# EndlessReform/smoltts

Hardware: AMD Instinct MI355X
Metric: Mimi frames/sec (=12.5 x RTF), greedy DualAR decode + Mimi decode to PCM (higher is better)
Workload: dtype bf16 weights, fp32 activations/accumulate, fp32 KV cache (LM); fp32 (Mimi)

## Files before the change

### smoltts_amd/csrc/argmax_dev.h

```cpp
#pragma once
#include "x3.h"

namespace smoltts {

struct Top2 {
  float v1;
  int i1;
  float v2;
};
__device__ __forceinline__ Top2 top2_merge(Top2 a, Top2 b) {
  Top2 o;
  const bool a_first = (a.v1 > b.v1) || (a.v1 == b.v1 && a.i1 < b.i1);
  if (a_first) {
    o.v1 = a.v1; o.i1 = a.i1; o.v2 = fmaxf(a.v2, b.v1);
  } else {
    o.v1 = b.v1; o.i1 = b.i1; o.v2 = fmaxf(b.v2, a.v1);
  }
  return o;
}

__device__ __forceinline__ uint32_t mix32(uint32_t x) {
  x ^= x >> 16; x *= 0x7feb352dU; x ^= x >> 15; x *= 0x846ca68bU; x ^= x >> 16;
  return x;
}
__device__ __forceinline__ float uniform01(uint64_t seed, int slot, int frame, int step, int col) {
  uint32_t h = mix32((uint32_t)seed ^ 0x9E3779B9U * (uint32_t)(slot + 1));
  h = mix32(h ^ (uint32_t)(seed >> 32) ^ 0x85EBCA6BU * (uint32_t)(frame + 1));
  h = mix32(h ^ 0xC2B2AE35U * (uint32_t)(step + 1));
  h = mix32(h ^ 0x27D4EB2FU * (uint32_t)(col + 1));
  return ((float)(h >> 8) + 0.5f) * (1.0f / 16777216.0f);
}

struct ArgmaxScratch {
  Top2 sh[4];
  Top2 sh2[4];
  int id;
};

struct FilterScratch {
  double m[2][4];
  int c[2][4];
};

template <int CTRL>
__device__ __forceinline__ uint32_t dpp_u32(uint32_t x) { return (uint32_t)__builtin_amdgcn_update_dpp(0, (int)x, CTRL, 0xF, 0xF, true); }
template <bool ROWS32>
__device__ __forceinline__ uint32_t swap_u32(uint32_t x, int lane) {
  const bool upper = (lane & (ROWS32 ? 32 : 16)) != 0;
  if (ROWS32) {
    const auto r = __builtin_amdgcn_permlane32_swap(x, x, false, false);
    return upper ? r[0] : r[1];
  }
  const auto r = __builtin_amdgcn_permlane16_swap(x, x, false, false);
  return upper ? r[0] : r[1];
}
__device__ __forceinline__ int wave_sum_i32(int x, int lane) {
  x += (int)dpp_u32<0xB1>(x);
  x += (int)dpp_u32<0x4E>(x);
  x += (int)dpp_u32<0x141>(x);
  x += (int)dpp_u32<0x140>(x);
  x += (int)swap_u32<false>(x, lane);
  x += (int)swap_u32<true>(x, lane);
  return x;
}
#define ST_F64_STEP(FETCH)                                                         \
  {                                                                                \
    const uint64_t b_ = (uint64_t)__double_as_longlong(x);                         \
    const uint32_t lo_ = FETCH((uint32_t)b_), hi_ = FETCH((uint32_t)(b_ >> 32));   \
    x += __longlong_as_double((long long)(((uint64_t)hi_ << 32) | lo_));           \
  }
__device__ __forceinline__ double wave_sum_f64(double x, int lane) {
#define ST_SWAP16(V) swap_u32<false>((V), lane)
#define ST_SWAP32(V) swap_u32<true>((V), lane)
  ST_F64_STEP(dpp_u32<0xB1>)
  ST_F64_STEP(dpp_u32<0x4E>)
  ST_F64_STEP(dpp_u32<0x141>)
  ST_F64_STEP(dpp_u32<0x140>)
  ST_F64_STEP(ST_SWAP16)
  ST_F64_STEP(ST_SWAP32)
#undef ST_SWAP16
#undef ST_SWAP32
  return x;
}
// ... 247 lines not shown
        wu = 0;
        for (int bit = 30; bit >= 0; --bit) {
          const uint32_t cand = wu | (1u << bit);
          double m = 0.0;
#define ST_ABOVE(V, Q) if (nz_bits(((V) - a.v1) * inv_t) < cand) m += (double)(Q);
#define ST_ABOVE_S(V, J) if (ord_key(V) >= tk) ST_ABOVE(V, mass_q(((V) - a.v1) * inv_t))
          if (vec) {
#pragma unroll
            for (int i = 0; i < 8; ++i) {
              ST_ABOVE(v[i].x, fq[i * 4]) ST_ABOVE(v[i].y, fq[i * 4 + 1]) ST_ABOVE(v[i].z, fq[i * 4 + 2]) ST_ABOVE(v[i].w, fq[i * 4 + 3])
            }
          } else {
            ST_SCOLS(ST_ABOVE_S)
          }
#undef ST_ABOVE_S
#undef ST_ABOVE
          if (wg_sum_f64(m, *F, round++, lane, wave) < P) wu = cand;
        }
      }
    }
    Top2 k{-INFINITY, 0x7fffffff, -INFINITY};
    float kz = 0.f;
#define ST_KEY(V, J)                                                  \
  {                                                                   \
    const float z = ((V) - a.v1) * inv_t;                   \
    if (z >= cut && (!FILTERS || nz_bits(z) <= wu)) {                 \
      const float u = uniform01(seed, key_slot, frame, sa.step, (J)); \
      const float key = z - logf(-logf(u));                           \
      if (key > k.v1) {                                               \
        k.v1 = key; k.i1 = (J);                                       \
        if constexpr (SCORE) kz = (V) - a.v1;                         \
      }                                                               \
    }                                                                 \
  }
#define ST_KEY_S(V, J) if (ord_key(V) >= tk) ST_KEY(V, J)
    if (vec) {
#pragma unroll
      for (int i = 0; i < 8; ++i) {
        const int j = tid * 4 + i * 1024;
        if (j < n_cols) { ST_KEY(v[i].x, j) ST_KEY(v[i].y, j + 1) ST_KEY(v[i].z, j + 2) ST_KEY(v[i].w, j + 3) }
      }
    } else if (FILTERS && fon) {
      ST_SCOLS(ST_KEY_S)
    } else {
      for (int j = tid; j < n_cols; j += 256) ST_KEY(ST_LFIX(row[j], j), j)
    }
#undef ST_KEY_S
#undef ST_KEY
    const int ki = k.i1;
#pragma unroll
    for (int o = 32; o > 0; o >>= 1) {
      Top2 b;
      b.v1 = __shfl_xor(k.v1, o); b.i1 = __shfl_xor(k.i1, o); b.v2 = -INFINITY;
      k = top2_merge(k, b);
    }
    if (lane == 0) S.sh2[wave] = k;
    __syncthreads();
    const Top2 w = top2_merge(top2_merge(S.sh2[0], S.sh2[1]), top2_merge(S.sh2[2], S.sh2[3]));
    a.i1 = w.i1;
    if constexpr (SCORE) {
      if (ki == w.i1) C->z = kz;
      __syncthreads();
      score_z = C->z;
    }
  }
#undef ST_SCOLS
#undef ST_SGROUP
#undef ST_LFIX
  if (a.i1 < 0 || a.i1 >= n_cols) a.i1 = 0;
  if (tid == 0) {
    if (temp <= 0.f && margin && (margin_mask == nullptr || margin_mask[r])) {
      const float gap = a.v1 - a.v2;
      if (gap < margin[r]) {
        margin[r] = gap;
        if (sa.margin_at) sa.margin_at[r] = (sa.frames ? sa.frames[r] : sa.frame_base + r) * 64 + sa.step;
      }
    }
  }
  if constexpr (SCORE)
    if (tid == 0) *lp_out = (float)((double)score_z - (log(score_s) - 40.0 * 0.6931471805599453094));
  return a.i1;
}

template <int CTRL>
__device__ __forceinline__ Top2 top2_dpp(Top2 t) {
  Top2 b;
  b.v1 = __int_as_float(__builtin_amdgcn_update_dpp(0, __float_as_int(t.v1), CTRL, 0xF, 0xF, true));
  b.i1 = __builtin_amdgcn_update_dpp(0, t.i1, CTRL, 0xF, 0xF, true);
  b.v2 = __int_as_float(__builtin_amdgcn_update_dpp(0, __float_as_int(t.v2), CTRL, 0xF, 0xF, true));
  return top2_merge(t, b);
}
template <bool ROWS32>
__device__ __forceinline__ Top2 top2_swap(Top2 t, int lane) {
  const unsigned a[3] = {__float_as_uint(t.v1), (unsigned)t.i1, __float_as_uint(t.v2)};
  unsigned o[3];
  const bool upper = (lane & (ROWS32 ? 32 : 16)) != 0;
#pragma unroll
  for (int i = 0; i < 3; ++i) {
    if (ROWS32) {
      const auto r = __builtin_amdgcn_permlane32_swap(a[i], a[i], false, false);
      o[i] = upper ? r[0] : r[1];
    } else {
      const auto r = __builtin_amdgcn_permlane16_swap(a[i], a[i], false, false);
      o[i] = upper ? r[0] : r[1];
    }
  }
  return top2_merge(t, Top2{__uint_as_float(o[0]), (int)o[1], __uint_as_float(o[2])});
}
__device__ __forceinline__ Top2 cand_pick_wave(const float* cand, int tiles, int lane) {
  Top2 t{-INFINITY, 0x7fffffff, -INFINITY};
  for (int j = lane; j < tiles; j += 64) {
    const float4 c = *reinterpret_cast<const float4*>(cand + (size_t)j * 4);
    t = top2_merge(t, Top2{c.x, __float_as_int(c.y), c.z});
  }
  t = top2_dpp<0xB1>(t);
  t = top2_dpp<0x4E>(t);
  t = top2_dpp<0x141>(t);
  t = top2_dpp<0x140>(t);
  t = top2_swap<false>(t, lane);
  t = top2_swap<true>(t, lane);
  return t;
}

struct QkvGather {
  const float* table;
  const float* rope;
  float* q_out;
  float* kc;
  float* vc;
  int n_q_heads, n_kv_heads, cache_len, pos;
};

__device__ __forceinline__ float4 rope_gathered4(float4 v, float4 cs) {
#pragma clang fp contract(off)
  const float o0 = v.x * cs.x - v.y * cs.y, o1 = v.y * cs.x + v.x * cs.y;
  const float o2 = v.z * cs.z - v.w * cs.w, o3 = v.w * cs.z + v.z * cs.w;
  return make_float4(o0, o1, o2, o3);
}

constexpr int QG_MAX = 2;
struct QkvRegs { float4 v[QG_MAX], cs[QG_MAX]; };

__device__ __forceinline__ void qkv_gather_load(const QkvGather& g, long erow, int base, QkvRegs& o) {
  const int qd = g.n_q_heads * 64, kd = g.n_kv_heads * 64, nqkv = qd + 2 * kd;
  const float* trow = g.table + erow * nqkv;
#pragma unroll
  for (int i = 0; i < QG_MAX; ++i) {
    const int n0 = base + (threadIdx.x + i * 256) * 4;
    o.v[i] = n0 < nqkv ? *reinterpret_cast<const float4*>(trow + n0) : make_float4(0.f, 0.f, 0.f, 0.f);
    o.cs[i] = n0 < qd + kd ? *reinterpret_cast<const float4*>(g.rope + ((long)g.pos * 32 + ((n0 & 63) >> 1)) * 2) : make_float4(1.f, 0.f, 1.f, 0.f);
  }
}

__device__ __forceinline__ void qkv_gather_store(const QkvGather& g, int r, int base, const QkvRegs& in) {
  const int qd = g.n_q_heads * 64, kd = g.n_kv_heads * 64, nqkv = qd + 2 * kd;
#pragma unroll
  for (int i = 0; i < QG_MAX; ++i) {
    const int n0 = base + (threadIdx.x + i * 256) * 4;
    if (n0 >= nqkv) continue;
    float4 v = in.v[i];
    if (n0 < qd + kd) v = rope_gathered4(v, in.cs[i]);
    if (n0 < qd) {
      *reinterpret_cast<float4*>(g.q_out + (long)r * qd + n0) = v;
    } else {
      const int nn = n0 - qd;
      float* dst = nn < kd ? g.kc : g.vc;
      const int h = (nn < kd ? nn : nn - kd) >> 6, d = nn & 63;
      *reinterpret_cast<float4*>(dst + (((long)r * g.n_kv_heads + h) * g.cache_len + g.pos) * 64 + d) = v;
    }
  }
}

}
```

### smoltts_amd/csrc/gemm3.hip

```cpp
#include <stdlib.h>

#include "argmax_dev.h"
#ifndef SMOLTTS_DBG_PIECES
#define SMOLTTS_DBG_PIECES 3
#endif
#ifndef SMOLTTS_DBG_PIECES_RESID
#define SMOLTTS_DBG_PIECES_RESID SMOLTTS_DBG_PIECES
#endif

namespace smoltts {

struct Gemm3Dev {
  const char* w;
  const float* wscale;
  const char* x3;
  int M, N, K;
  int w_nt;
  int f8_act;
  int half_rows;
  const float* ssq_in;
  float eps;
  const float* bias;
  const float* resid;
  float* out;
// ... 480 lines not shown
  b = __builtin_amdgcn_cvt_scalef32_pk_fp8_bf16(b, __builtin_bit_cast(bf16x2_t, v.w), 1.0f, true);
  return make_uint2(__builtin_bit_cast(unsigned, a), __builtin_bit_cast(unsigned, b));
}

template <int NTW, int EPI>
__global__ __launch_bounds__(256) void gemm3_rows_f8_kernel(Gemm3Dev p) {
  __shared__ uint2 xs[4 * 64];
  const int tid = threadIdx.x, wave = tid >> 6, lane = tid & 63;
  const int r = lane & 15, q = lane >> 4;
  const int nchunks = p.K >> 5;
  const int mtile0 = blockIdx.y * 4;
  const int tile0 = (blockIdx.x * 4 + wave) * NTW;
  const char* sp = ((mtile0 + wave) * 16 < p.M) ? p.x3 + (size_t)(mtile0 + wave) * nchunks * 3072 + lane * 16 : nullptr;
  const char* wb[NTW];
  bool wv[NTW];
#pragma unroll
  for (int t = 0; t < NTW; ++t) {
    wv[t] = (tile0 + t) * 16 < p.N;
    wb[t] = p.w + (size_t)(tile0 + t) * nchunks * 512 + lane * 8;
  }
  f32x4 acc[NTW][4];
#pragma unroll
  for (int t = 0; t < NTW; ++t)
#pragma unroll
    for (int mt = 0; mt < 4; ++mt) acc[t][mt] = (f32x4){0.f, 0.f, 0.f, 0.f};
  uint4 stage;
  uint2 wnext[NTW];
  auto fetch = [&](int c) {
    stage = sp ? *reinterpret_cast<const uint4*>(sp + (size_t)c * 3072) : make_uint4(0, 0, 0, 0);
#pragma unroll
    for (int t = 0; t < NTW; ++t) wnext[t] = wv[t] ? *reinterpret_cast<const uint2*>(wb[t] + (size_t)c * 512) : make_uint2(0, 0);
  };
  fetch(0);
  for (int c = 0; c < nchunks; ++c) {
    __syncthreads();
    xs[tid] = bf16x8_to_fp8x8(stage);
    long a[NTW];
#pragma unroll
    for (int t = 0; t < NTW; ++t) a[t] = __builtin_bit_cast(long, wnext[t]);
    __syncthreads();
    if (c + 1 < nchunks) fetch(c + 1);
#pragma unroll
    for (int mt = 0; mt < 4; ++mt) {
      const long b = __builtin_bit_cast(long, xs[mt * 64 + lane]);
#pragma unroll
      for (int t = 0; t < NTW; ++t) acc[t][mt] = __builtin_amdgcn_mfma_f32_16x16x32_fp8_fp8(a[t], b, acc[t][mt], 0, 0, 0);
    }
  }
  rows_epilogue<NTW, EPI, true>(p, acc, mtile0, tile0, r, q);
}

__device__ __forceinline__ float dpp_ror8(float x) {
  return __int_as_float(__builtin_amdgcn_update_dpp(0, __float_as_int(x), 0x128, 0xF, 0xF, true));
}
__device__ __forceinline__ float row8_sum(float x) {
  x += __int_as_float(__builtin_amdgcn_update_dpp(0, __float_as_int(x), 0xB1, 0xF, 0xF, true));
  x += __int_as_float(__builtin_amdgcn_update_dpp(0, __float_as_int(x), 0x4E, 0xF, 0xF, true));
  x += __int_as_float(__builtin_amdgcn_update_dpp(0, __float_as_int(x), 0x141, 0xF, 0xF, true));
  return x;
}
__device__ __forceinline__ void swap16(float& a, float& b) {
  const auto r = __builtin_amdgcn_permlane16_swap(__float_as_uint(a), __float_as_uint(b), false, false);
  a = __uint_as_float(r[0]);
  b = __uint_as_float(r[1]);
}
__device__ __forceinline__ void dot4x2(float4 a, float4 b, float4 k0, float4 k1, float& lo, float& hi) {
  lo = a.x * k0.x; lo = fmaf(a.y, k0.y, lo); lo = fmaf(a.z, k0.z, lo); lo = fmaf(a.w, k0.w, lo);
  hi = b.x * k1.x; hi = fmaf(b.y, k1.y, hi); hi = fmaf(b.z, k1.z, hi); hi = fmaf(b.w, k1.w, hi);
}
__device__ __forceinline__ float score16(float4 a, float4 b, float4 k0, float4 k1) {
  float lo, hi;
  dot4x2(a, b, k0, k1, lo, hi);
  return row8_sum(lo) + row8_sum(hi);
}

#ifndef SMOLTTS_DBG_AWO_ORDER
#define SMOLTTS_DBG_AWO_ORDER 1
#endif
constexpr int AWO_R = 2;

template <int G, bool TWO>
struct AwoUnit {
  float4 ka0, kb0, va0, vb0, ka1, kb1, va1, vb1, qa[G], qb[G];
  int rl, kvc;
  bool hv, ok0, ok1;
};

template <int G, bool TWO, bool PICK>
__device__ __forceinline__ void awo_load(AwoUnit<G, TWO>& u, const Gemm3Dev& p, int unit, int kv_pairs, int row0, int lane, long erow = 0,
                                         bool write_kv = false) {
  const int kq = lane >> 5, jj = (lane >> 3) & 3, hb = jj & 1, m8 = lane & 7;
  const int L = p.a_pos + 1;
  u.rl = unit / kv_pairs;
  const int kvh = (unit - u.rl * kv_pairs) * 2 + kq, row = row0 + u.rl;
  u.hv = kvh < p.n_kv_heads;
  u.kvc = u.hv ? kvh : p.n_kv_heads - 1;
  const long cb = (((long)row * p.n_kv_heads + u.kvc) * p.cache_len) * 64 + 4 * m8;
  u.ok0 = jj < L;
  u.ok1 = TWO && jj + 4 < L;
  const long o0 = cb + (long)(u.ok0 ? jj : 0) * 64, o1 = cb + (long)(u.ok1 ? jj + 4 : 0) * 64;
  const float *k0p = p.kc + o0, *v0p = p.vc + o0, *k1p = p.kc + o1, *v1p = p.vc + o1;
  const int qd = p.n_q_heads * 64, kd = p.n_kv_heads * 64;
  const float* trow = PICK ? p.pk_table + erow * (qd + 2 * kd) : nullptr;
  const bool new0 = PICK && jj == p.a_pos, new1 = PICK && TWO && jj + 4 == p.a_pos;
  if (PICK) {
    const float *tk = trow + qd + u.kvc * 64 + 4 * m8, *tv = trow + qd + kd + u.kvc * 64 + 4 * m8;
    if (new0) { k0p = tk; v0p = tv; }
    if (new1) { k1p = tk; v1p = tv; }
  }
  u.ka0 = *reinterpret_cast<const float4*>(k0p); u.kb0 = *reinterpret_cast<const float4*>(k0p + 32);
  u.va0 = *reinterpret_cast<const float4*>(v0p + 32 * hb); u.vb0 = *reinterpret_cast<const float4*>(v0p + 32 * (1 - hb));
  if (TWO) {
    u.ka1 = *reinterpret_cast<const float4*>(k1p); u.kb1 = *reinterpret_cast<const float4*>(k1p + 32);
    u.va1 = *reinterpret_cast<const float4*>(v1p + 32 * hb); u.vb1 = *reinterpret_cast<const float4*>(v1p + 32 * (1 - hb));
  }
#pragma unroll
  for (int g = 0; g < G; ++g) {
    const float* qp = PICK ? trow + (u.kvc * G + g) * 64 + 4 * m8 : p.aq + (long)row * qd + (u.kvc * G + g) * 64 + 4 * m8;
    u.qa[g] = *reinterpret_cast<const float4*>(qp);
    u.qb[g] = *reinterpret_cast<const float4*>(qp + 32);
  }
  if (PICK) {
    const float4 csa = *reinterpret_cast<const float4*>(p.pk_rope + ((long)p.a_pos * 32 + 2 * m8) * 2);
    const float4 csb = *reinterpret_cast<const float4*>(p.pk_rope + ((long)p.a_pos * 32 + 16 + 2 * m8) * 2);
#pragma unroll
    for (int g = 0; g < G; ++g) { u.qa[g] = rope_gathered4(u.qa[g], csa); u.qb[g] = rope_gathered4(u.qb[g], csb); }
    const float4 ra0 = rope_gathered4(u.ka0, csa), rb0 = rope_gathered4(u.kb0, csb);
    if (new0) { u.ka0 = ra0; u.kb0 = rb0; }
    if (TWO) {
      const float4 ra1 = rope_gathered4(u.ka1, csa), rb1 = rope_gathered4(u.kb1, csb);
      if (new1) { u.ka1 = ra1; u.kb1 = rb1; }
    }
    if (write_kv && u.hv && (new0 || new1)) {
      float* kw = p.kc + cb + (long)p.a_pos * 64;
      float* vw = p.vc + cb + (long)p.a_pos * 64;
      const float4 ka = new0 ? u.ka0 : u.ka1, kb = new0 ? u.kb0 : u.kb1, va = new0 ? u.va0 : u.va1, vb = new0 ? u.vb0 : u.vb1;
      *reinterpret_cast<float4*>(kw) = ka; *reinterpret_cast<float4*>(kw + 32) = kb;
      *reinterpret_cast<float4*>(vw + 32 * hb) = va; *reinterpret_cast<float4*>(vw + 32 * (1 - hb)) = vb;
    }
  }
}

template <int G, bool TWO>
__device__ __forceinline__ void awo_compute(const AwoUnit<G, TWO>& u, char* frag, int lane) {
#pragma clang fp contract(off)
  constexpr int R = AWO_R;
  const int hb = (lane >> 3) & 1, m8 = lane & 7;
  const bool up = (lane & 16) != 0;
#pragma unroll
  for (int g = 0; g < G; ++g) {
    const float4 a = make_float4(u.qa[g].x * 0.125f, u.qa[g].y * 0.125f, u.qa[g].z * 0.125f, u.qa[g].w * 0.125f);
    const float4 b = make_float4(u.qb[g].x * 0.125f, u.qb[g].y * 0.125f, u.qb[g].z * 0.125f, u.qb[g].w * 0.125f);
    float s0 = score16(a, b, u.ka0, u.kb0), s1 = -INFINITY;
    s0 = u.ok0 ? s0 : -INFINITY;
    if (TWO) {
      s1 = score16(a, b, u.ka1, u.kb1);
      s1 = u.ok1 ? s1 : -INFINITY;
    }
    float mx = TWO ? fmaxf(s0, s1) : s0;
    mx = fmaxf(mx, dpp_ror8(mx));
    {
      float t = mx;
      swap16(mx, t);
      mx = fmaxf(mx, t);
    }
    const float e0 = __expf(s0 - mx);
    float den = e0;
    float4 oa = make_float4(e0 * u.va0.x, e0 * u.va0.y, e0 * u.va0.z, e0 * u.va0.w);
    float4 ob = make_float4(e0 * u.vb0.x, e0 * u.vb0.y, e0 * u.vb0.z, e0 * u.vb0.w);
    if (TWO) {
      const float e1 = __expf(s1 - mx);
      den += e1;
      oa.x = fmaf(e1, u.va1.x, oa.x); oa.y = fmaf(e1, u.va1.y, oa.y); oa.z = fmaf(e1, u.va1.z, oa.z); oa.w = fmaf(e1, u.va1.w, oa.w);
      ob.x = fmaf(e1, u.vb1.x, ob.x); ob.y = fmaf(e1, u.vb1.y, ob.y); ob.z = fmaf(e1, u.vb1.z, ob.z); ob.w = fmaf(e1, u.vb1.w, ob.w);
    }
    den += dpp_ror8(den);
    {
      float t = den;
      swap16(den, t);
      den += t;
    }
    oa.x += dpp_ror8(ob.x); oa.y += dpp_ror8(ob.y); oa.z += dpp_ror8(ob.z); oa.w += dpp_ror8(ob.w);
    swap16(oa.x, oa.z);
    swap16(oa.y, oa.w);
    const float inv = 1.0f / den;
    const float ox = (oa.x + oa.z) * inv, oy = (oa.y + oa.w) * inv;
    uint32_t h, mm, l;
    split3_pair(ox, oy, h, mm, l);
    const int c = 2 * (u.kvc * G + g) + hb;
    char* fp = frag + ((size_t)((c * 3) * 4 + (m8 >> 1)) * R + u.rl) * 16 + (m8 & 1) * 8 + (up ? 4 : 0);
    if (u.hv) {
      *reinterpret_cast<uint32_t*>(fp) = h;
      *reinterpret_cast<uint32_t*>(fp + 4 * R * 16) = mm;
      *reinterpret_cast<uint32_t*>(fp + 8 * R * 16) = l;
    }
  }
}

constexpr int AWO_NA = 4, AWO_NB = 8, AWO_U = 3;

template <int G, int T, bool TWO, bool W8, bool PICK, int NBF>
__global__ __launch_bounds__(768) void attn_wo_kernel(const char* w_, const float* kc_, const float* vc_, const float* q_or_cand, const float* pk_table_,
                                                      int m_tiles, int N_, int K_, int heads_pos, Gemm3Dev p) {
  KernargTouch<AWO_KERNARG_LINES> kt;
  kernarg_touch(kt);
  p.w = w_; p.kc = const_cast<float*>(kc_); p.vc = const_cast<float*>(vc_); p.pk_table = pk_table_;
  if (PICK) p.pk_cand = q_or_cand; else p.aq = q_or_cand;
  p.M = m_tiles & 0xffff; p.pk_tiles = m_tiles >> 16; p.N = N_; p.K = K_;
  p.n_q_heads = heads_pos & 255; p.n_kv_heads = (heads_pos >> 8) & 255; p.cache_len = (heads_pos >> 16) & 255; p.a_pos = heads_pos >> 24;
  constexpr int WTILE = W8 ? 512 : 1024, WLANE = W8 ? 8 : 16;
  constexpr int R = AWO_R, NA = AWO_NA, NB = AWO_NB, U = AWO_U;
  extern __shared__ __attribute__((aligned(16))) float smem[];
  const int tid = threadIdx.x, wave = __builtin_amdgcn_readfirstlane(tid >> 6), lane = tid & 63;
  const int r = lane & 15, q = lane >> 4;
  const int ng = blockIdx.x, row0 = blockIdx.y * R;
  const int nchunks = p.K >> 5;
  constexpr bool FULL = NBF != 0;
  const int nb = FULL ? NBF : ((nchunks + 2) / 3 < 1 ? 1 : ((nchunks + 2) / 3 > NB ? NB : (nchunks + 2) / 3));
  char* frag = reinterpret_cast<char*>(smem);
  float4* red4 = reinterpret_cast<float4*>(frag + (size_t)nchunks * 3 * 4 * R * 16);
  lds_poison(smem, (size_t)nchunks * 3 * 4 * R * 16 + (size_t)NB * T * 1024);
  STAMP3(0);

  if (wave < NA) {
    const int kv_pairs = (p.n_kv_heads + 1) >> 1;
    const int n_units = (p.M - row0 < R ? p.M - row0 : R) * kv_pairs;
    long erow0 = 0, erow1 = 0;
    Top2 t0{0.f, 0, 0.f}, t1 = t0;
#if SMOLTTS_DBG_AWO_ORDER
    if (PICK) __syncthreads();
#endif
    if (PICK) {
      const int n_cols = p.pk_tiles * 16;
      t0 = cand_pick_wave(p.pk_cand + (size_t)row0 * p.pk_tiles * 4, p.pk_tiles, lane);
      t1 = t0;
      if (row0 + 1 < p.M) t1 = cand_pick_wave(p.pk_cand + (size_t)(row0 + 1) * p.pk_tiles * 4, p.pk_tiles, lane);
      if (t0.i1 < 0 || t0.i1 >= n_cols) t0.i1 = 0;
      if (t1.i1 < 0 || t1.i1 >= n_cols) t1.i1 = 0;
      erow0 = (long)t0.i1 + p.pk_off;
      erow1 = (long)t1.i1 + p.pk_off;
    }
    AwoUnit<G, TWO> un;
    if (wave < n_units) awo_load<G, TWO, PICK>(un, p, wave, kv_pairs, row0, lane, wave / kv_pairs ? erow1 : erow0, blockIdx.x == 0);
    kernarg_touched(kt);
    const bool fin = wave < T;
    const int tf = fin ? wave : 0;
    const int m = row0 + r;
    const bool row_on = r < R;
    const bool mvalid = fin && row_on && m < p.M;
    float4 rr, bb, ga, gb, ws;
    rr = bb = make_float4(0.f, 0.f, 0.f, 0.f);
    ga = gb = ws = make_float4(1.f, 1.f, 1.f, 1.f);
    if (fin) {
      const int mc = m < p.M ? m : p.M - 1;
      const int n0r = (ng * T + tf) * 16 + q * 4;
      const int n0 = n0r < p.N ? n0r : p.N - 4;
      if (W8) ws = *reinterpret_cast<const float4*>(p.wscale + n0);
      if (PICK) {
        const uint2 e = *reinterpret_cast<const uint2*>(p.pk_emb + ((r & 1) ? erow1 : erow0) * p.K + n0);
        rr = make_float4(bf16_lo(e.x), bf16_hi(e.x), bf16_lo(e.y), bf16_hi(e.y));
      } else {
        rr = *reinterpret_cast<const float4*>(p.resid + (long)mc * p.ldo + n0);
      }
      if (p.bias != nullptr) bb = *reinterpret_cast<const float4*>(p.bias + n0);
      if (p.emit.x3a && p.emit.gamma_a) ga = *reinterpret_cast<const float4*>(p.emit.gamma_a + n0);
      if (p.emit.x3b && p.emit.gamma_b) gb = *reinterpret_cast<const float4*>(p.emit.gamma_b + n0);
    }
    STAMP3(5);
#if SMOLTTS_DBG_AWO_ORDER
    if (!PICK) __syncthreads();
#endif
    if (wave < n_units) awo_compute(un, frag, lane);
    for (int unit = wave + NA; unit < n_units; unit += NA) {
      awo_load<G, TWO, PICK>(un, p, unit, kv_pairs, row0, lane, unit / kv_pairs ? erow1 : erow0, blockIdx.x == 0);
      awo_compute(un, frag, lane);
    }
    STAMP3(6);
    __syncthreads();
    __syncthreads();
    STAMP3(3);
    if (PICK && blockIdx.x == 0 && wave == NA - 1 && lane == 0) {
#pragma unroll
      for (int rl = 0; rl < R; ++rl) {
        const int row = row0 + rl;
        if (row >= p.M) break;
        const Top2 t = rl ? t1 : t0;
        p.pk_ids[(long)row * p.pk_ids_stride] = t.i1;
        if (p.pk_margin && (p.pk_mask == nullptr || p.pk_mask[row])) {
          const float gap = t.v1 - t.v2;
          if (gap < p.pk_margin[row]) {
            p.pk_margin[row] = gap;
            if (p.pk_margin_at) p.pk_margin_at[row] = p.pk_frames[row] * 64 + p.pk_step;
          }
        }
      }
    }
    if (!fin) return;
    float4 part[NB];
#pragma unroll
    for (int w = 0; w < NB; ++w) part[w] = red4[((w < nb ? w : 0) * T + tf) * 64 + lane];
    float v[4] = {0.f, 0.f, 0.f, 0.f};
#pragma unroll
    for (int w = 0; w < NB; ++w) {
      const bool on = w < nb;
      v[0] += on ? part[w].x : 0.f;
      v[1] += on ? part[w].y : 0.f;
      v[2] += on ? part[w].z : 0.f;
      v[3] += on ? part[w].w : 0.f;
    }
    const int ntile = ng * T + tf;
    const int n0 = ntile * 16 + q * 4;
    const bool valid = mvalid && n0 < p.N;
    if (W8) { v[0] *= ws.x; v[1] *= ws.y; v[2] *= ws.z; v[3] *= ws.w; }
    v[0] = v[0] + bb.x + rr.x; v[1] = v[1] + bb.y + rr.y; v[2] = v[2] + bb.z + rr.z; v[3] = v[3] + bb.w + rr.w;
    if (valid) {
      *reinterpret_cast<float4*>(p.out + (long)m * p.ldo + n0) = make_float4(v[0], v[1], v[2], v[3]);
      if (p.emit.x3a) x3_emit4(p.emit.x3a, m, n0, p.N >> 5, v[0] * ga.x, v[1] * ga.y, v[2] * ga.z, v[3] * ga.w);
      if (p.emit.x3b) x3_emit4(p.emit.x3b, m, n0, p.N >> 5, v[0] * gb.x, v[1] * gb.y, v[2] * gb.z, v[3] * gb.w);
    }
    if (p.emit.ssq) {
      float sq = valid ? ((v[0] * v[0] + v[1] * v[1]) + (v[2] * v[2] + v[3] * v[3])) : 0.f;
      sq = sum_xor16_32(sq);
      if (q == 0 && mvalid && ntile * 16 < p.N) p.emit.ssq[(size_t)m * (p.N >> 4) + ntile] = sq;
    }
    STAMP3(4);
    return;
  }

  const int gw = wave - NA;
#if SMOLTTS_DBG_AWO_ORDER
  __syncthreads();
#endif
  uint4 wf[U][T];
#pragma unroll
  for (int u = 0; u < U; ++u) {
    const int c = gw + u * nb;
#pragma unroll
    for (int t = 0; t < T; ++t) {
      const int ntile = ng * T + t;
      wf[u][t] = (FULL ? (NBF == NB || gw < nb) : (gw < nb && c < nchunks && ntile * 16 < p.N)) ? load_wfrag<W8, false>(p.w + ((size_t)ntile * nchunks + c) * WTILE + lane * WLANE)
                                                             : make_uint4(0, 0, 0, 0);
    }
  }
  kernarg_touched(kt);
  STAMP3(5);
  __syncthreads();
  f32x4 acc[T];
#pragma unroll
  for (int t = 0; t < T; ++t) acc[t] = (f32x4){0.f, 0.f, 0.f, 0.f};
// ... 260 lines not shown
```

### smoltts_amd/csrc/lm_engine.hip

```cpp
#include <stdlib.h>
#include <string.h>

#include <algorithm>
#include <new>

#include "argmax_dev.h"
#include "embed_dev.h"

using namespace smoltts;

struct SmolttsEngine {
  SmolttsLMConfig cfg;
  SmolttsLMWeights w;
  const char* arena;
  size_t arena_bytes;
  const float* fast_qkv;
};

constexpr int STAGE_RING = 8;
constexpr int GRAPH_FORMS = 64;
constexpr int FORM_SLOW = 1, FORM_FAST = 2, FORM_FILTER = 4, FORM_LENGTH = 8, FORM_SCORE = 16, FORM_ALIGN = 32;
enum GraphKind { GRAPH_FRAME, GRAPH_TAIL, GRAPH_MULTI, GRAPH_KINDS };

struct PinnedRing {
// ... 136 lines not shown
  for (int i = b; i < ATT_SPLIT_MAX_PAIRS; i += gridDim.x * blockDim.x) attn_ticket[i] = 0;
  if (b >= B) return;
  margin_at[b] = 0;
  iota[b] = b;
  for (int i = 0; i < n_fast; ++i) fastpos[i * B + b] = i;
  pos[b] = 0; frames[b] = 0; done[b] = 1; mask[b] = 0; salt[b] = 0;
  margin[b] = INFINITY;
  for (int i = 0; i <= n_fast; ++i) { cur_col[b * (1 + n_fast) + i] = 0; new_col[b * (1 + n_fast) + i] = 0; }
}

template <typename Entry>
__global__ void slot_scatter_kernel(int n, const Entry* entries, const int* slots, Entry* table) {
  const int i = blockIdx.x * blockDim.x + threadIdx.x;
  if (i < n) table[slots[i]] = entries[i];
}

__global__ void slot_reset_kernel(int B, int n_slots, const int* slots, const int* last_row, const int* row_pos, int* pos,
                                  int* frames, int* done, int* mask, float* margin, int* salt) {
  const int b = blockIdx.x * blockDim.x + threadIdx.x;
  if (b >= B) return;
  int hit = -1;
  for (int i = 0; i < n_slots; ++i)
    if (slots[i] == b) hit = i;
  mask[b] = hit >= 0;
  if (hit >= 0) {
    pos[b] = row_pos[last_row[hit]] + 1;
    frames[b] = 0; done[b] = 0; margin[b] = INFINITY;
    salt[b] += 1;
  }
}

__global__ void slot_start_kernel(int B, int H, int n_slots, const int* slots, const int* last_row, const int* row_pos,
                                  const int* grid, int* pos, int* frames, int* done, float* margin, int* cur_col, int* salt) {
  const int b = blockIdx.x * blockDim.x + threadIdx.x;
  if (b >= B) return;
  for (int i = 0; i < n_slots; ++i)
    if (slots[i] == b) {
      const int lr = last_row[i];
      pos[b] = row_pos[lr];
      frames[b] = 0; done[b] = 0; margin[b] = INFINITY;
      salt[b] += 1;
      for (int k = 0; k < H; ++k) cur_col[b * H + k] = grid[(long)lr * H + k];
    }
}

__global__ void slot_park_kernel(int B, int n_slots, const int* slots, const int* last_row, const int* row_pos, int* pos,
                                 int* done, int* mask) {
  const int b = blockIdx.x * blockDim.x + threadIdx.x;
  if (b >= B) return;
  for (int i = 0; i < n_slots; ++i)
    if (slots[i] == b) { pos[b] = row_pos[last_row[i]] + 1; done[b] = 1; mask[b] = 0; }
}

__global__ void slot_parkpos_kernel(int B, int n_slots, const int* slots, const int* where, int* pos, int* done, int* mask) {
  const int b = blockIdx.x * blockDim.x + threadIdx.x;
  if (b >= B) return;
  for (int i = 0; i < n_slots; ++i)
    if (slots[i] == b) { pos[b] = where[i]; done[b] = 1; mask[b] = 0; }
}

struct CommitArgs {
  int B, H, max_frames, max_seq, im_end, stop_on_eos, advance_pos, do_commit;
  int* new_col;
  int *mask, *cur_col, *codes, *pos, *frames, *done;
  const float* slow_logits; int slow_cols; SampleArgs slow_sa;
  const float* last_logits; int last_cols; SampleArgs last_sa;
  float* margin;
  const float* slow_cand; int slow_tiles;
  const float* last_cand; int last_tiles;
  float* logprob;
  int* attn_ticket;
};

template <bool FILTERS, bool LENGTH, bool SCORE>
__global__ __launch_bounds__(256) void commit_embed_kernel(CommitArgs a, EmbedTables t, float* xt, EmitDev emit) {
  __shared__ int s_col[64];
  __shared__ float sh4[4];
  __shared__ ArgmaxScratch s_pick[2];
  const int b = blockIdx.x, tid = threadIdx.x, H = a.H;
  if (b == 0 && a.attn_ticket)
    for (int i = tid; i < ATT_SPLIT_MAX_PAIRS; i += blockDim.x) a.attn_ticket[i] = 0;
  int id_slow = 0, id_last = 0;
  const bool c_slow = a.slow_logits && a.slow_cand, c_last = a.last_logits && a.last_cand;
  if (c_slow || c_last) {
    __shared__ int s_id[2];
    __shared__ float s_gap[2];
    const int wave = tid >> 6, lane = tid & 63;
    if ((wave == 0 && c_slow) || (wave == 1 && c_last)) {
      const float* cand = wave == 0 ? a.slow_cand + (size_t)b * a.slow_tiles * 4 : a.last_cand + (size_t)b * a.last_tiles * 4;
      Top2 t = cand_pick_wave(cand, wave == 0 ? a.slow_tiles : a.last_tiles, lane);
      if (t.i1 < 0 || t.i1 >= (wave == 0 ? a.slow_cols : a.last_cols)) t.i1 = 0;
      if (lane == 0) { s_id[wave] = t.i1; s_gap[wave] = t.v1 - t.v2; }
    }
    __syncthreads();
    if (tid == 0 && a.margin && a.mask[b]) {
#pragma unroll
      for (int k = 0; k < 2; ++k) {
        if (!(k == 0 ? c_slow : c_last)) continue;
        const SampleArgs& sa = k == 0 ? a.slow_sa : a.last_sa;
        if (s_gap[k] < a.margin[b]) {
          a.margin[b] = s_gap[k];
          if (sa.margin_at) sa.margin_at[b] = (sa.frames ? sa.frames[b] : sa.frame_base + b) * 64 + sa.step;
        }
      }
    }
    if (c_slow) id_slow = s_id[0];
    if (c_last) id_last = s_id[1];
  }
  float lp_slow = 0.f;
  ScoreScratch* sc = nullptr;
  if constexpr (SCORE) {
    __shared__ ScoreScratch s_score;
    sc = &s_score;
  }
  if constexpr (FILTERS) {
    __shared__ FilterScratch s_filt[2];
    if (a.slow_logits && !c_slow) id_slow = argmax_row<true, LENGTH, SCORE>(a.slow_logits + (long)b * a.slow_cols, a.slow_cols, (a.slow_cols & 3) == 0, b, a.margin, a.mask, a.slow_sa, s_pick[0], &s_filt[0], sc, &lp_slow);
    if (a.last_logits && !c_last) id_last = argmax_row<true>(a.last_logits + (long)b * a.last_cols, a.last_cols, (a.last_cols & 3) == 0, b, a.margin, a.mask, a.last_sa, s_pick[1], &s_filt[1]);
  } else {
    if (a.slow_logits && !c_slow) id_slow = argmax_row<false, LENGTH, SCORE>(a.slow_logits + (long)b * a.slow_cols, a.slow_cols, (a.slow_cols & 3) == 0, b, a.margin, a.mask, a.slow_sa, s_pick[0], nullptr, sc, &lp_slow);
    if (a.last_logits && !c_last) id_last = argmax_row(a.last_logits + (long)b * a.last_cols, a.last_cols, (a.last_cols & 3) == 0, b, a.margin, a.mask, a.last_sa, s_pick[1]);
  }
  int f = 0;
  bool live = false;
  if (tid < 64) { f = a.frames[b]; live = a.do_commit && a.mask[b]; }
  const bool publish = live && f < a.max_frames;
  int slow_now = 0;
  if (tid < H) {
    int nv = a.new_col[b * H + tid];
    if (a.slow_logits && tid == 0) nv = id_slow;
    if (a.last_logits && tid == H - 1) nv = id_last;
    if ((a.slow_logits && tid == 0) || (a.last_logits && tid == H - 1)) a.new_col[b * H + tid] = nv;
    const int v = publish ? nv : a.cur_col[b * H + tid];
    s_col[tid] = v;
    if (publish) {
      a.cur_col[b * H + tid] = v;
      a.codes[((long)b * a.max_frames + f) * H + tid] = v;
      if constexpr (SCORE) {
        if (tid == 0 && a.logprob && a.slow_logits && !c_slow) a.logprob[(long)b * a.max_frames + f] = lp_slow;
      }
    }
  }
  slow_now = a.slow_logits ? id_slow : a.new_col[b * H];
  if (tid == 0) {
    int d = a.done[b];
    if (live) {
      int p = a.pos[b];
      if (a.advance_pos) a.pos[b] = ++p;
      if (publish) a.frames[b] = f + 1;
      if ((a.stop_on_eos && slow_now == a.im_end) || f + 1 >= a.max_frames || p >= a.max_seq) a.done[b] = d = 1;
    }
    a.mask[b] = !d;
  }
  __syncthreads();
  embed_row(t, s_col, b, xt, emit, sh4);
}

SmolttsGemm3Args base3(int fmt, const void* w, const void* x3, int M, int N, int K, int epilogue) {
  SmolttsGemm3Args a;
  memset(&a, 0, sizeof(a));
  a.w_dev = w; a.x3_dev = x3; a.M = M; a.N = N; a.K = K; a.epilogue = epilogue;
  a.w_format = fmt;
  if (fmt == SMOLTTS_W_FP8) a.w_scale_dev = reinterpret_cast<const float*>(static_cast<const char*>(w) + (size_t)N * K);
  return a;
}

bool dup_hit(const SmolttsSession* s, int code, int N) { return s->dup_code == code && (s->dup_n <= 0 || s->dup_n == N); }

int launch_gemm3_m(const SmolttsSession* s, const SmolttsGemm3Args& a, hipStream_t st) {
  ST_TRY(launch_gemm3(a, st));
  if (a.epilogue != SMOLTTS_EPI_RESID && dup_hit(s, a.epilogue, a.N)) ST_TRY(launch_gemm3(a, st));
  return SMOLTTS_OK;
}

int run_block(const SmolttsSession* s, const SmolttsBlockWeights& bw, int dim, int n_head, int n_kv, int inter, float* x,
              float* q, int M, const int* row_pos, const int* row_slot, const float* rope, void* kc, void* vc,
              int cache_len, const char* in_x3, const EmitArgs& next, hipStream_t st, bool first_pos = false,
              int kv_format = SMOLTTS_KV_F32, int iota_pos = -1, bool qkv_done = false, int w_stream = 0,
              const SmolttsPickArgs* pick = nullptr) {
  const SmolttsEngine* e = s->e;
  const char* A = e->arena;
  const float eps = e->cfg.norm_eps;
  if (!qkv_done) {
    SmolttsGemm3Args a = base3(e->cfg.weight_format, A + bw.wqkv, in_x3, M, (n_head + 2 * n_kv) * 64, dim, SMOLTTS_EPI_QKV_ROPE);
    a.fp8_activations = s->fp8_prefill;
    a.ssq_in_dev = s->ssq; a.eps = eps; a.out_dev = q; a.ldo = n_head * 64;
    a.rope_dev = rope; a.row_pos_dev = row_pos; a.row_slot_dev = row_slot;
    a.k_cache_dev = (float*)kc; a.v_cache_dev = (float*)vc; a.n_q_heads = n_head; a.n_kv_heads = n_kv; a.cache_len = cache_len;
    a.kv_format = kv_format; a.w_stream = (w_stream & (1 | SMOLTTS_STREAM_W_DEPTH_QKVO)) != 0;
    if (first_pos) a.v_x3_dev = s->x3a;
    ST_TRY(launch_gemm3_m(s, a, st));
  }
  const bool fused_attn = !first_pos && iota_pos > 0 && s->fuse_depth_attn && kv_format == SMOLTTS_KV_F32 &&
                          smoltts_gemm3_attn_fusable(n_head, n_kv, cache_len) && dim == n_head * 64;
  if (!first_pos && !fused_attn) {
    const int reps = dup_hit(s, cache_len <= 16 ? 100 : 101, 0) ? 2 : 1;
    for (int i = 0; i < reps; ++i)
      ST_TRY(launch_attention(q, kc, vc, row_pos, row_slot, M, n_head, n_kv, cache_len, 0, nullptr, s->x3a, st, kv_format, iota_pos,
                              s->split_attn ? s->attn_part : nullptr, s->attn_ticket));
  }
  {
    SmolttsGemm3Args a = base3(e->cfg.weight_format, A + bw.wo, s->x3a, M, dim, dim, SMOLTTS_EPI_RESID);
    a.fp8_activations = s->fp8_prefill;
    a.resid_dev = x; a.out_dev = x; a.ldo = dim;
    a.emit_a_dev = s->x3n; a.gamma_a_dev = (const float*)(A + bw.ffn_norm); a.ssq_out_dev = s->ssq; a.w_stream = (w_stream & (1 | SMOLTTS_STREAM_W_DEPTH_QKVO)) != 0;
    if (fused_attn) {
      a.attn_q_dev = q; a.attn_pos = iota_pos; a.k_cache_dev = (float*)kc; a.v_cache_dev = (float*)vc;
      a.n_q_heads = n_head; a.n_kv_heads = n_kv; a.cache_len = cache_len; a.kv_format = SMOLTTS_KV_F32;
      a.pick = pick;
    }
    ST_REQUIRE(pick == nullptr || fused_attn, SMOLTTS_E_STATE, "run_block: a pick needs the fused depth attention");
    ST_TRY(launch_gemm3(a, st));
  }
  {
    SmolttsGemm3Args a = base3(e->cfg.weight_format, A + bw.w13, s->x3n, M, 2 * inter, dim, SMOLTTS_EPI_SWIGLU);
    a.fp8_activations = s->fp8_prefill;
    a.ssq_in_dev = s->ssq; a.eps = eps; a.x3_out_dev = s->x3h; a.w_stream = (w_stream & (1 | SMOLTTS_STREAM_W_DEPTH_W13)) != 0;
    ST_TRY(launch_gemm3_m(s, a, st));
  }
  {
    SmolttsGemm3Args a = base3(e->cfg.weight_format, A + bw.w2, s->x3h, M, dim, inter, SMOLTTS_EPI_RESID);
    a.fp8_activations = s->fp8_prefill;
    a.resid_dev = x; a.out_dev = x; a.ldo = dim;
    a.emit_a_dev = next.x3a; a.gamma_a_dev = next.gamma_a; a.emit_b_dev = next.x3b; a.gamma_b_dev = next.gamma_b;
    a.ssq_out_dev = next.ssq; a.w_stream = (w_stream & (1 | SMOLTTS_STREAM_W_DEPTH_W2)) != 0;
    ST_TRY(launch_gemm3(a, st));
  }
  return SMOLTTS_OK;
}

// ... 1234 lines not shown
```

Baseline: 28590.

## Prefetch candidate tiles and KV/state loads ahead of the argmax reduction

The candidate-argmax pick is split into a load phase, which issues a fixed number of float4 candidate reads per lane up front, and a merge phase that reduces them later. This lets other independent loads (KV cache rows, rope tables, epilogue vectors, per-row state like frames/mask/pos) be issued in between and overlap with the candidate fetch latency. The attention load is likewise split into early (KV, rope) and late (picked-embedding q/k/v) parts so only the dependent part waits on the argmax result. It also switches the top-2 merge to a select-based form and caches row state in registers, at the cost of more register pressure and duplicated tail-handling logic.

```diff
diff --git a/smoltts_amd/csrc/argmax_dev.h b/smoltts_amd/csrc/argmax_dev.h
--- a/smoltts_amd/csrc/argmax_dev.h
+++ b/smoltts_amd/csrc/argmax_dev.h
@@ -1,4 +1,5 @@
 #pragma once
+#include "cand_index.h"
 #include "x3.h"
 
 namespace smoltts {
@@ -412,13 +413,21 @@
   return a.i1;
 }
 
+__device__ __forceinline__ Top2 top2_merge_sel(Top2 a, Top2 b) {
+  const bool a_first = (a.v1 > b.v1) || (a.v1 == b.v1 && a.i1 < b.i1);
+  Top2 o;
+  o.v1 = a_first ? a.v1 : b.v1;
+  o.i1 = a_first ? a.i1 : b.i1;
+  o.v2 = fmaxf(a_first ? a.v2 : b.v2, a_first ? b.v1 : a.v1);
+  return o;
+}
 template <int CTRL>
 __device__ __forceinline__ Top2 top2_dpp(Top2 t) {
   Top2 b;
   b.v1 = __int_as_float(__builtin_amdgcn_update_dpp(0, __float_as_int(t.v1), CTRL, 0xF, 0xF, true));
   b.i1 = __builtin_amdgcn_update_dpp(0, t.i1, CTRL, 0xF, 0xF, true);
   b.v2 = __int_as_float(__builtin_amdgcn_update_dpp(0, __float_as_int(t.v2), CTRL, 0xF, 0xF, true));
-  return top2_merge(t, b);
+  return top2_merge_sel(t, b);
 }
 template <bool ROWS32>
 __device__ __forceinline__ Top2 top2_swap(Top2 t, int lane) {
@@ -435,21 +444,43 @@
       o[i] = upper ? r[0] : r[1];
     }
   }
-  return top2_merge(t, Top2{__uint_as_float(o[0]), (int)o[1], __uint_as_float(o[2])});
-}
-__device__ __forceinline__ Top2 cand_pick_wave(const float* cand, int tiles, int lane) {
-  Top2 t{-INFINITY, 0x7fffffff, -INFINITY};
-  for (int j = lane; j < tiles; j += 64) {
-    const float4 c = *reinterpret_cast<const float4*>(cand + (size_t)j * 4);
-    t = top2_merge(t, Top2{c.x, __float_as_int(c.y), c.z});
-  }
-  t = top2_dpp<0xB1>(t);
-  t = top2_dpp<0x4E>(t);
-  t = top2_dpp<0x141>(t);
-  t = top2_dpp<0x140>(t);
-  t = top2_swap<false>(t, lane);
-  t = top2_swap<true>(t, lane);
-  return t;
+  return top2_merge_sel(t, Top2{__uint_as_float(o[0]), (int)o[1], __uint_as_float(o[2])});
+}
+struct CandRegs { float4 c[CAND_ROUNDS]; };
+__device__ __forceinline__ void cand_pick_load(const float* cand, int tiles, int lane, CandRegs& o) {
+#pragma unroll
+  for (int i = 0; i < CAND_ROUNDS; ++i)
+    o.c[i] = *reinterpret_cast<const float4*>(cand + (size_t)cand_round_read(lane, i, tiles) * 4);
+}
+template <int NR>
+__device__ __forceinline__ void cand_pick_merge(const float* const (&cand)[NR], int tiles, int lane, const CandRegs (&in)[NR], Top2 (&t)[NR]) {
+#pragma unroll
+  for (int r = 0; r < NR; ++r) t[r] = Top2{-INFINITY, 0x7fffffff, -INFINITY};
+#pragma unroll
+  for (int i = 0; i < CAND_ROUNDS; ++i) {
+    const bool on = cand_round_on(lane, i, tiles);
+#pragma unroll
+    for (int r = 0; r < NR; ++r) {
+      const Top2 m = top2_merge_sel(t[r], Top2{in[r].c[i].x, __float_as_int(in[r].c[i].y), in[r].c[i].z});
+      t[r].v1 = on ? m.v1 : t[r].v1; t[r].i1 = on ? m.i1 : t[r].i1; t[r].v2 = on ? m.v2 : t[r].v2;
+    }
+  }
+  for (int j = cand_tail_first(lane); j < tiles; j += CAND_LANES) {
+    float4 c[NR];
+#pragma unroll
+    for (int r = 0; r < NR; ++r) c[r] = *reinterpret_cast<const float4*>(cand[r] + (size_t)j * 4);
+#pragma unroll
+    for (int r = 0; r < NR; ++r) t[r] = top2_merge_sel(t[r], Top2{c[r].x, __float_as_int(c[r].y), c[r].z});
+  }
+#define ST_BFLY(STEP)                  \
+  _Pragma("unroll") for (int r = 0; r < NR; ++r) t[r] = STEP;
+  ST_BFLY(top2_dpp<0xB1>(t[r]))
+  ST_BFLY(top2_dpp<0x4E>(t[r]))
+  ST_BFLY(top2_dpp<0x141>(t[r]))
+  ST_BFLY(top2_dpp<0x140>(t[r]))
+  ST_BFLY(top2_swap<false>(t[r], lane))
+  ST_BFLY(top2_swap<true>(t[r], lane))
+#undef ST_BFLY
 }
 
 struct QkvGather {
diff --git a/smoltts_amd/csrc/cand_index.h b/smoltts_amd/csrc/cand_index.h
--- /dev/null
+++ b/smoltts_amd/csrc/cand_index.h
@@ -0,0 +1,19 @@
+#pragma once
+
+#if defined(__HIPCC__) || defined(__CUDACC__)
+#define ST_CAND_HD __host__ __device__ inline __attribute__((always_inline))
+#else
+#define ST_CAND_HD inline
+#endif
+
+namespace smoltts {
+
+constexpr int CAND_LANES = 64;
+constexpr int CAND_ROUNDS = 4;
+
+ST_CAND_HD int cand_round_tile(int lane, int i) { return lane + i * CAND_LANES; }
+ST_CAND_HD bool cand_round_on(int lane, int i, int tiles) { return cand_round_tile(lane, i) < tiles; }
+ST_CAND_HD int cand_round_read(int lane, int i, int tiles) { return cand_round_on(lane, i, tiles) ? cand_round_tile(lane, i) : tiles - 1; }
+ST_CAND_HD int cand_tail_first(int lane) { return lane + CAND_ROUNDS * CAND_LANES; }
+
+}
diff --git a/smoltts_amd/csrc/gemm3.hip b/smoltts_amd/csrc/gemm3.hip
--- a/smoltts_amd/csrc/gemm3.hip
+++ b/smoltts_amd/csrc/gemm3.hip
@@ -586,13 +586,13 @@
 template <int G, bool TWO>
 struct AwoUnit {
   float4 ka0, kb0, va0, vb0, ka1, kb1, va1, vb1, qa[G], qb[G];
+  float4 csa, csb;
   int rl, kvc;
   bool hv, ok0, ok1;
 };
 
 template <int G, bool TWO, bool PICK>
-__device__ __forceinline__ void awo_load(AwoUnit<G, TWO>& u, const Gemm3Dev& p, int unit, int kv_pairs, int row0, int lane, long erow = 0,
-                                         bool write_kv = false) {
+__device__ __forceinline__ void awo_load_early(AwoUnit<G, TWO>& u, const Gemm3Dev& p, int unit, int kv_pairs, int row0, int lane) {
   const int kq = lane >> 5, jj = (lane >> 3) & 3, hb = jj & 1, m8 = lane & 7;
   const int L = p.a_pos + 1;
   u.rl = unit / kv_pairs;
@@ -602,22 +602,34 @@
   const long cb = (((long)row * p.n_kv_heads + u.kvc) * p.cache_len) * 64 + 4 * m8;
   u.ok0 = jj < L;
   u.ok1 = TWO && jj + 4 < L;
-  const long o0 = cb + (long)(u.ok0 ? jj : 0) * 64, o1 = cb + (long)(u.ok1 ? jj + 4 : 0) * 64;
+  const bool new0 = PICK && jj == p.a_pos, new1 = PICK && TWO && jj + 4 == p.a_pos;
+  const long o0 = cb + (long)(u.ok0 && !new0 ? jj : 0) * 64, o1 = cb + (long)(u.ok1 && !new1 ? jj + 4 : 0) * 64;
   const float *k0p = p.kc + o0, *v0p = p.vc + o0, *k1p = p.kc + o1, *v1p = p.vc + o1;
-  const int qd = p.n_q_heads * 64, kd = p.n_kv_heads * 64;
-  const float* trow = PICK ? p.pk_table + erow * (qd + 2 * kd) : nullptr;
-  const bool new0 = PICK && jj == p.a_pos, new1 = PICK && TWO && jj + 4 == p.a_pos;
-  if (PICK) {
-    const float *tk = trow + qd + u.kvc * 64 + 4 * m8, *tv = trow + qd + kd + u.kvc * 64 + 4 * m8;
-    if (new0) { k0p = tk; v0p = tv; }
-    if (new1) { k1p = tk; v1p = tv; }
-  }
   u.ka0 = *reinterpret_cast<const float4*>(k0p); u.kb0 = *reinterpret_cast<const float4*>(k0p + 32);
   u.va0 = *reinterpret_cast<const float4*>(v0p + 32 * hb); u.vb0 = *reinterpret_cast<const float4*>(v0p + 32 * (1 - hb));
   if (TWO) {
     u.ka1 = *reinterpret_cast<const float4*>(k1p); u.kb1 = *reinterpret_cast<const float4*>(k1p + 32);
     u.va1 = *reinterpret_cast<const float4*>(v1p + 32 * hb); u.vb1 = *reinterpret_cast<const float4*>(v1p + 32 * (1 - hb));
   }
+  if (PICK) {
+    u.csa = *reinterpret_cast<const float4*>(p.pk_rope + ((long)p.a_pos * 32 + 2 * m8) * 2);
+    u.csb = *reinterpret_cast<const float4*>(p.pk_rope + ((long)p.a_pos * 32 + 16 + 2 * m8) * 2);
+  }
+}
+
+template <int G, bool TWO, bool PICK>
+__device__ __forceinline__ void awo_load_late(AwoUnit<G, TWO>& u, const Gemm3Dev& p, int row0, int lane, long erow = 0, bool write_kv = false) {
+  const int jj = (lane >> 3) & 3, hb = jj & 1, m8 = lane & 7;
+  const int row = row0 + u.rl;
+  const int qd = p.n_q_heads * 64, kd = p.n_kv_heads * 64;
+  const float* trow = PICK ? p.pk_table + erow * (qd + 2 * kd) : nullptr;
+  const bool new0 = PICK && jj == p.a_pos, new1 = PICK && TWO && jj + 4 == p.a_pos;
+  float4 tka, tkb, tva, tvb;
+  if (PICK) {
+    const float *tk = trow + qd + u.kvc * 64 + 4 * m8, *tv = trow + qd + kd + u.kvc * 64 + 4 * m8;
+    tka = *reinterpret_cast<const float4*>(tk); tkb = *reinterpret_cast<const float4*>(tk + 32);
+    tva = *reinterpret_cast<const float4*>(tv + 32 * hb); tvb = *reinterpret_cast<const float4*>(tv + 32 * (1 - hb));
+  }
 #pragma unroll
   for (int g = 0; g < G; ++g) {
     const float* qp = PICK ? trow + (u.kvc * G + g) * 64 + 4 * m8 : p.aq + (long)row * qd + (u.kvc * G + g) * 64 + 4 * m8;
@@ -625,24 +637,29 @@
     u.qb[g] = *reinterpret_cast<const float4*>(qp + 32);
   }
   if (PICK) {
-    const float4 csa = *reinterpret_cast<const float4*>(p.pk_rope + ((long)p.a_pos * 32 + 2 * m8) * 2);
-    const float4 csb = *reinterpret_cast<const float4*>(p.pk_rope + ((long)p.a_pos * 32 + 16 + 2 * m8) * 2);
+    const float4 csa = u.csa, csb = u.csb;
 #pragma unroll
     for (int g = 0; g < G; ++g) { u.qa[g] = rope_gathered4(u.qa[g], csa); u.qb[g] = rope_gathered4(u.qb[g], csb); }
-    const float4 ra0 = rope_gathered4(u.ka0, csa), rb0 = rope_gathered4(u.kb0, csb);
-    if (new0) { u.ka0 = ra0; u.kb0 = rb0; }
+    const float4 ra = rope_gathered4(tka, csa), rb = rope_gathered4(tkb, csb);
+    if (new0) { u.ka0 = ra; u.kb0 = rb; u.va0 = tva; u.vb0 = tvb; }
     if (TWO) {
-      const float4 ra1 = rope_gathered4(u.ka1, csa), rb1 = rope_gathered4(u.kb1, csb);
-      if (new1) { u.ka1 = ra1; u.kb1 = rb1; }
+      if (new1) { u.ka1 = ra; u.kb1 = rb; u.va1 = tva; u.vb1 = tvb; }
     }
     if (write_kv && u.hv && (new0 || new1)) {
+      const long cb = (((long)row * p.n_kv_heads + u.kvc) * p.cache_len) * 64 + 4 * m8;
       float* kw = p.kc + cb + (long)p.a_pos * 64;
       float* vw = p.vc + cb + (long)p.a_pos * 64;
-      const float4 ka = new0 ? u.ka0 : u.ka1, kb = new0 ? u.kb0 : u.kb1, va = new0 ? u.va0 : u.va1, vb = new0 ? u.vb0 : u.vb1;
-      *reinterpret_cast<float4*>(kw) = ka; *reinterpret_cast<float4*>(kw + 32) = kb;
-      *reinterpret_cast<float4*>(vw + 32 * hb) = va; *reinterpret_cast<float4*>(vw + 32 * (1 - hb)) = vb;
-    }
-  }
+      *reinterpret_cast<float4*>(kw) = ra; *reinterpret_cast<float4*>(kw + 32) = rb;
+      *reinterpret_cast<float4*>(vw + 32 * hb) = tva; *reinterpret_cast<float4*>(vw + 32 * (1 - hb)) = tvb;
+    }
+  }
+}
+
+template <int G, bool TWO, bool PICK>
+__device__ __forceinline__ void awo_load(AwoUnit<G, TWO>& u, const Gemm3Dev& p, int unit, int kv_pairs, int row0, int lane, long erow = 0,
+                                         bool write_kv = false) {
+  awo_load_early<G, TWO, PICK>(u, p, unit, kv_pairs, row0, lane);
+  awo_load_late<G, TWO, PICK>(u, p, row0, lane, erow, write_kv);
 }
 
 template <int G, bool TWO>
@@ -734,18 +751,21 @@
 #if SMOLTTS_DBG_AWO_ORDER
     if (PICK) __syncthreads();
 #endif
+    const float* cand0 = p.pk_cand + (size_t)row0 * p.pk_tiles * 4;
+    const bool lone = row0 + 1 >= p.M;
+    const float* cand1 = lone ? cand0 : cand0 + (size_t)p.pk_tiles * 4;
+    const float* const cands[2] = {cand0, cand1};
+    CandRegs cr[2];
     if (PICK) {
-      const int n_cols = p.pk_tiles * 16;
-      t0 = cand_pick_wave(p.pk_cand + (size_t)row0 * p.pk_tiles * 4, p.pk_tiles, lane);
-      t1 = t0;
-      if (row0 + 1 < p.M) t1 = cand_pick_wave(p.pk_cand + (size_t)(row0 + 1) * p.pk_tiles * 4, p.pk_tiles, lane);
-      if (t0.i1 < 0 || t0.i1 >= n_cols) t0.i1 = 0;
-      if (t1.i1 < 0 || t1.i1 >= n_cols) t1.i1 = 0;
-      erow0 = (long)t0.i1 + p.pk_off;
-      erow1 = (long)t1.i1 + p.pk_off;
+      cand_pick_load(cand0, p.pk_tiles, lane, cr[0]);
+      cand_pick_load(cand1, p.pk_tiles, lane, cr[1]);
     }
     AwoUnit<G, TWO> un;
-    if (wave < n_units) awo_load<G, TWO, PICK>(un, p, wave, kv_pairs, row0, lane, wave / kv_pairs ? erow1 : erow0, blockIdx.x == 0);
+    if (PICK) {
+      if (wave < n_units) awo_load_early<G, TWO, PICK>(un, p, wave, kv_pairs, row0, lane);
+    } else {
+      if (wave < n_units) awo_load<G, TWO, PICK>(un, p, wave, kv_pairs, row0, lane);
+    }
     kernarg_touched(kt);
     const bool fin = wave < T;
     const int tf = fin ? wave : 0;
@@ -755,20 +775,28 @@
     float4 rr, bb, ga, gb, ws;
     rr = bb = make_float4(0.f, 0.f, 0.f, 0.f);
     ga = gb = ws = make_float4(1.f, 1.f, 1.f, 1.f);
+    const int n0r_f = (ng * T + tf) * 16 + q * 4;
+    const int n0_f = n0r_f < p.N ? n0r_f : p.N - 4;
     if (fin) {
       const int mc = m < p.M ? m : p.M - 1;
-      const int n0r = (ng * T + tf) * 16 + q * 4;
-      const int n0 = n0r < p.N ? n0r : p.N - 4;
-      if (W8) ws = *reinterpret_cast<const float4*>(p.wscale + n0);
-      if (PICK) {
-        const uint2 e = *reinterpret_cast<const uint2*>(p.pk_emb + ((r & 1) ? erow1 : erow0) * p.K + n0);
-        rr = make_float4(bf16_lo(e.x), bf16_hi(e.x), bf16_lo(e.y), bf16_hi(e.y));
-      } else {
-        rr = *reinterpret_cast<const float4*>(p.resid + (long)mc * p.ldo + n0);
-      }
-      if (p.bias != nullptr) bb = *reinterpret_cast<const float4*>(p.bias + n0);
-      if (p.emit.x3a && p.emit.gamma_a) ga = *reinterpret_cast<const float4*>(p.emit.gamma_a + n0);
-      if (p.emit.x3b && p.emit.gamma_b) gb = *reinterpret_cast<const float4*>(p.emit.gamma_b + n0);
+      if (W8) ws = *reinterpret_cast<const float4*>(p.wscale + n0_f);
+      if (!PICK) rr = *reinterpret_cast<const float4*>(p.resid + (long)mc * p.ldo + n0_f);
+      if (p.bias != nullptr) bb = *reinterpret_cast<const float4*>(p.bias + n0_f);
+      if (p.emit.x3a && p.emit.gamma_a) ga = *reinterpret_cast<const float4*>(p.emit.gamma_a + n0_f);
+      if (p.emit.x3b && p.emit.gamma_b) gb = *reinterpret_cast<const float4*>(p.emit.gamma_b + n0_f);
+    }
+    if (PICK) {
+      const int n_cols = p.pk_tiles * 16;
+      Top2 tt[2];
+      cand_pick_merge<2>(cands, p.pk_tiles, lane, cr, tt);
+      t0 = tt[0]; t1 = tt[1];
+      if (t0.i1 < 0 || t0.i1 >= n_cols) t0.i1 = 0;
+      if (t1.i1 < 0 || t1.i1 >= n_cols) t1.i1 = 0;
+      erow0 = (long)t0.i1 + p.pk_off;
+      erow1 = (long)t1.i1 + p.pk_off;
+      const uint2 e = *reinterpret_cast<const uint2*>(p.pk_emb + ((r & 1) ? erow1 : erow0) * p.K + n0_f);
+      if (wave < n_units) awo_load_late<G, TWO, PICK>(un, p, row0, lane, wave / kv_pairs ? erow1 : erow0, blockIdx.x == 0);
+      if (fin) rr = make_float4(bf16_lo(e.x), bf16_hi(e.x), bf16_lo(e.y), bf16_hi(e.y));
     }
     STAMP3(5);
 #if SMOLTTS_DBG_AWO_ORDER
diff --git a/smoltts_amd/csrc/lm_engine.hip b/smoltts_amd/csrc/lm_engine.hip
--- a/smoltts_amd/csrc/lm_engine.hip
+++ b/smoltts_amd/csrc/lm_engine.hip
@@ -242,24 +242,38 @@
     for (int i = tid; i < ATT_SPLIT_MAX_PAIRS; i += blockDim.x) a.attn_ticket[i] = 0;
   int id_slow = 0, id_last = 0;
   const bool c_slow = a.slow_logits && a.slow_cand, c_last = a.last_logits && a.last_cand;
-  if (c_slow || c_last) {
+  const bool cp = c_slow || c_last;
+  int f_pre = 0, mask_pre = 0, nv_pre = 0, cv_pre = 0, done_pre = 0, pos_pre = 0;
+  float margin_pre = 0.f;
+  if (cp) {
     __shared__ int s_id[2];
     __shared__ float s_gap[2];
     const int wave = tid >> 6, lane = tid & 63;
-    if ((wave == 0 && c_slow) || (wave == 1 && c_last)) {
-      const float* cand = wave == 0 ? a.slow_cand + (size_t)b * a.slow_tiles * 4 : a.last_cand + (size_t)b * a.last_tiles * 4;
-      Top2 t = cand_pick_wave(cand, wave == 0 ? a.slow_tiles : a.last_tiles, lane);
-      if (t.i1 < 0 || t.i1 >= (wave == 0 ? a.slow_cols : a.last_cols)) t.i1 = 0;
-      if (lane == 0) { s_id[wave] = t.i1; s_gap[wave] = t.v1 - t.v2; }
-    }
+    const bool picker = (wave == 0 && c_slow) || (wave == 1 && c_last);
+    const bool slow_row = c_slow && (wave == 0 || !c_last);
+    const int tiles = slow_row ? a.slow_tiles : a.last_tiles;
+    const float* cand = slow_row ? a.slow_cand + (size_t)b * a.slow_tiles * 4 : a.last_cand + (size_t)b * a.last_tiles * 4;
+    if (a.margin) margin_pre = a.margin[b];
+    const float* const cands[1] = {cand};
+    CandRegs cr[1];
+    cand_pick_load(cand, tiles, lane, cr[0]);
+    const int hc = tid < H ? tid : H - 1;
+    f_pre = a.frames[b]; mask_pre = a.mask[b];
+    nv_pre = a.new_col[b * H + hc]; cv_pre = a.cur_col[b * H + hc];
+    done_pre = a.done[b]; pos_pre = a.pos[b];
+    Top2 tt[1];
+    cand_pick_merge<1>(cands, tiles, lane, cr, tt);
+    Top2 t = tt[0];
+    if (t.i1 < 0 || t.i1 >= (slow_row ? a.slow_cols : a.last_cols)) t.i1 = 0;
+    if (picker && lane == 0) { s_id[wave] = t.i1; s_gap[wave] = t.v1 - t.v2; }
     __syncthreads();
-    if (tid == 0 && a.margin && a.mask[b]) {
+    if (tid == 0 && a.margin && mask_pre) {
 #pragma unroll
       for (int k = 0; k < 2; ++k) {
         if (!(k == 0 ? c_slow : c_last)) continue;
         const SampleArgs& sa = k == 0 ? a.slow_sa : a.last_sa;
-        if (s_gap[k] < a.margin[b]) {
-          a.margin[b] = s_gap[k];
+        if (s_gap[k] < margin_pre) {
+          a.margin[b] = margin_pre = s_gap[k];
           if (sa.margin_at) sa.margin_at[b] = (sa.frames ? sa.frames[b] : sa.frame_base + b) * 64 + sa.step;
         }
       }
@@ -283,15 +297,18 @@
   }
   int f = 0;
   bool live = false;
-  if (tid < 64) { f = a.frames[b]; live = a.do_commit && a.mask[b]; }
+  if (tid < 64) {
+    if (cp) { f = f_pre; live = a.do_commit && mask_pre; }
+    else { f = a.frames[b]; live = a.do_commit && a.mask[b]; }
+  }
   const bool publish = live && f < a.max_frames;
   int slow_now = 0;
   if (tid < H) {
-    int nv = a.new_col[b * H + tid];
+    int nv = cp ? nv_pre : a.new_col[b * H + tid];
     if (a.slow_logits && tid == 0) nv = id_slow;
     if (a.last_logits && tid == H - 1) nv = id_last;
     if ((a.slow_logits && tid == 0) || (a.last_logits && tid == H - 1)) a.new_col[b * H + tid] = nv;
-    const int v = publish ? nv : a.cur_col[b * H + tid];
+    const int v = publish ? nv : (cp ? cv_pre : a.cur_col[b * H + tid]);
     s_col[tid] = v;
     if (publish) {
       a.cur_col[b * H + tid] = v;
@@ -303,9 +320,9 @@
   }
   slow_now = a.slow_logits ? id_slow : a.new_col[b * H];
   if (tid == 0) {
-    int d = a.done[b];
+    int d = cp ? done_pre : a.done[b];
     if (live) {
-      int p = a.pos[b];
+      int p = cp ? pos_pre : a.pos[b];
       if (a.advance_pos) a.pos[b] = ++p;
       if (publish) a.frames[b] = f + 1;
       if ((a.stop_on_eos && slow_now == a.im_end) || f + 1 >= a.max_frames || p >= a.max_seq) a.done[b] = d = 1;
```

Result: no change. 28840 (median of 6 runs) (+0.9%).
